# mpc001/auto_avsr

Measured on AMD Instinct MI355X. Metric: video-frames/sec/node (25fps 88x88, max-frames=1600), E2E training step (fwd+bwd+clip+AdamW), higher is better.
Workload: dtype f16 activations x f16x2 weights (atrunk3, atrunk4, decoder, encoder, trunk3, trunk4) + split-bf16 (everything else) forward / bf16 backward

## Files before the change

### auto_avsr_amd/csrc/gemm_core.h

```cpp
#pragma once
#include <algorithm>
#include "prims.h"

namespace avsr_gemm_impl {

struct Params {
    const void* A;
    const void* B;
    const void* B2;
    int lda, ldb;
    int M, N, K;
    int k_chunk;
    const float* bias;
    int act;
    const void* gate;
    int gate_dtype, ldg;
    float gate_scale;
    float drop_p;
    uint64_t seed;
    float alpha;
    const float* alpha_dev;
    const uint64_t* seed_dev;
    const float* resid;
    int ldr;
    void* C;
    void* C2;
    int ldc2;
    int c_dtype, ldc;
    int accumulate;
    int nsplit, batch_h, nbatch;
    long sAb, sAh, sBb, sBh, sCb, sCh;
    int a_skew, skew_off, skew_lim;
    int resid_dtype;
    int cH, cW, cC;
    int cOH, cOW;
    int cKH, cKW, cS, cPH, cPW;
    int cT, cKT, cPT;
    float* colsum;
    float* colstat;
    int colstat_rows;
    float* colsum_a;
    int cN, xcd_order, ncls;
    int k_rot;
    int cls_tile0[5], cls_py[4], cls_px[4], cls_y0[4], cls_x0[4], cls_h[4], cls_w[4], cls_nkh[4], cls_nkw[4];
};

template <class T> struct Raw8;
template <> struct Raw8<bf16_t> {
    bf16x8 v;
    AVSR_DEV void zero() { v = bf16x8{0, 0, 0, 0, 0, 0, 0, 0}; }
    AVSR_DEV void load(const bf16_t* p) { v = *reinterpret_cast<const bf16x8*>(p); }
    AVSR_DEV void set(int e, const bf16_t* p) { v[e] = (short)*p; }
    AVSR_DEV float get(int e) const { return bf2f((bf16_t)v[e]); }
};
template <> struct Raw8<float> {
    f32x4 a, b;
    AVSR_DEV void zero() { a = f32x4{0, 0, 0, 0}; b = a; }
    AVSR_DEV void load(const float* p) {
        a = *reinterpret_cast<const f32x4*>(p);
        b = *reinterpret_cast<const f32x4*>(p + 4);
    }
    AVSR_DEV void set(int e, const float* p) {
        if (e < 4) a[e] = *p; else b[e - 4] = *p;
    }
    AVSR_DEV float get(int e) const { return e < 4 ? a[e] : b[e - 4]; }
};
// ... 556 lines not shown
```

### auto_avsr_amd/csrc/gemm_fast.hip

```cpp
#include "gemm_fast_kernel.h"
#include "gemm_pair.h"
#include "avsr_hip.h"

namespace {

using avsr_gemm_impl::Params;

#define g_tune avsr_tune_knobs

using avsr_fast::FastKernel;

template <int BM, int BN, int STAGES, int CV, int WGM, int WGN, int ABL, int KS, int F16 = 0, int WP = 1>
__global__ __launch_bounds__(64 * WGM * WGN * KS) void gemm_fast_kernel(Params p) {
    AVSR_DYN_SMEM(smem);
    FastKernel<BM, BN, STAGES, CV, WGM, WGN, ABL, KS, F16, WP>::run(p, smem);
}

template <int BM, int BN, int STAGES, int CV = 0, int WGM = 2, int WGN = 2, int ABL = 0, int KS = 1, int F16 = 0, int WP = 1>
void launch_fast(Params& p, int split_k, hipStream_t stream) {
    using K = FastKernel<BM, BN, STAGES, CV, WGM, WGN, ABL, KS, F16, WP>;
    p.k_rot = CV == 0 ? g_tune[7] : 0;
    p.xcd_order = g_tune[1] == 0 ? (CV == 0 && BM == 64 && BN == 64) : (g_tune[1] == 1);
    int gy;
    if (CV == 0) {
        int kc = (p.K + split_k - 1) / split_k;
        kc = ((kc + 63) / 64) * 64;
        split_k = (p.K + kc - 1) / kc;
        p.k_chunk = kc;
        gy = (p.M + BM - 1) / BM;
    } else {
        split_k = 1;
        int t0 = 0;
        for (int c = 0; c < p.ncls; c++) {
            p.cls_tile0[c] = t0;
            t0 += (int)(((long)p.cN * p.cls_h[c] * p.cls_w[c] + BM - 1) / BM);
        }
        p.cls_tile0[p.ncls] = t0;
        gy = t0;
    }
    dim3 grid((p.N + BN - 1) / BN, gy, split_k), block(K::NTHR);
    AVSR_LAUNCH((gemm_fast_kernel<BM, BN, STAGES, CV, WGM, WGN, ABL, KS, F16, WP>), grid, block, K::LDS_BYTES, stream, p);
}

template <int CV>
bool launch_tile(int tile, Params& p, int split_k, hipStream_t stream) {
    switch (tile) {
        case 1: if (CV == 0) { launch_fast<64, 64, 3, 0>(p, split_k, stream); return true; } return false;
        case 2: launch_fast<128, 64, 3, CV>(p, split_k, stream); return true;
        case 3:
            if (CV == 1 && g_tune[2] == 1) launch_fast<128, 128, 3, 1, 2, 2, 1>(p, split_k, stream);
            else if (CV == 1 && g_tune[2] == 2) launch_fast<128, 128, 3, 1, 2, 2, 2>(p, split_k, stream);
// ... 20 lines not shown

template <int CV>
bool launch_tile_h16(int tile, Params& p, int split_k, hipStream_t stream) {
    switch (tile) {
        case 1: if (CV == 0) { launch_fast<64, 64, 3, 0, 2, 2, 0, 1, 1>(p, split_k, stream); return true; } return false;
        case 4: launch_fast<128, 128, 2, CV, 2, 2, 0, 1, 1>(p, split_k, stream); return true;
        case 7: launch_fast<128, 64, 2, CV, 2, 2, 0, 1, 1>(p, split_k, stream); return true;
        default: return false;
    }
}

template <int CV>
bool launch_tile_h16x2(int tile, Params& p, int split_k, hipStream_t stream) {
    switch (tile) {
        case 1: if (CV == 0) { launch_fast<64, 64, 3, 0, 2, 2, 0, 1, 1, 2>(p, split_k, stream); return true; } return false;
        case 21: if (CV == 0) { launch_fast<64, 64, 2, 0, 2, 2, 0, 1, 1, 2>(p, split_k, stream); return true; } return false;
        case 4: launch_fast<128, 128, 2, CV, 2, 2, 0, 1, 1, 2>(p, split_k, stream); return true;
        case 7: launch_fast<128, 64, 2, CV, 2, 2, 0, 1, 1, 2>(p, split_k, stream); return true;
        case 2: launch_fast<128, 64, 3, CV, 2, 2, 0, 1, 1, 2>(p, split_k, stream); return true;
        case 5: launch_fast<256, 128, 2, CV, 4, 2, 0, 1, 1, 2>(p, split_k, stream); return true;
        case 8: launch_fast<256, 64, 2, CV, 4, 2, 0, 1, 1, 2>(p, split_k, stream); return true;
        case 22: launch_fast<128, 128, 2, CV, 2, 4, 0, 1, 1, 2>(p, split_k, stream); return true;
        case 23: launch_fast<256, 64, 3, CV, 4, 2, 0, 1, 1, 2>(p, split_k, stream); return true;
        case 31: if (CV == 0) { launch_fast<64, 64, 3, 0, 2, 2, 1, 1, 1, 2>(p, split_k, stream); return true; } return false;
        case 32: if (CV == 0) { launch_fast<64, 64, 3, 0, 2, 2, 2, 1, 1, 2>(p, split_k, stream); return true; } return false;
        case 33: if (CV == 0) { launch_fast<128, 64, 2, 0, 2, 2, 1, 1, 1, 2>(p, split_k, stream); return true; } return false;
        case 34: if (CV == 0) { launch_fast<128, 64, 2, 0, 2, 2, 2, 1, 1, 2>(p, split_k, stream); return true; } return false;
        case 35: if (CV == 0) { launch_fast<256, 128, 2, 0, 4, 2, 1, 1, 1, 2>(p, split_k, stream); return true; } return false;
        case 36: if (CV == 0) { launch_fast<256, 128, 2, 0, 4, 2, 2, 1, 1, 2>(p, split_k, stream); return true; } return false;
        default: return false;
    }
}

}

int avsr_conv_patch_supported(int N, int H, int W, int Cg, int Cout_eff, int KH, int KW, int stride, int pad_h, int pad_w);
int avsr_conv_patch_launch(int mode, const void* src, const void* w, const void* w_lo, int ldw, const void* resid, void* out, void* out2,
                           const void* zero_page, int N, int H, int W, int Cg, int Cout_eff, hipStream_t stream);
int avsr_conv3x3_c64_supported(int H, int W);
int avsr_conv3x3_c64_launch(int flip, const void* src, const void* wq, const void* resid, void* out, const void* zero_page, int N,
                            int H, int W, hipStream_t stream);

static int gemm16_nt_impl(int f16, const void* A, int lda, const void* B, const void* B_lo, int ldb, int M, int N, int K, const float* bias,
                          int act, const void* gate, int gate_dtype, int ldg, float gate_scale, float drop_p,
                          uint64_t seed, const uint64_t* seed_dev, float alpha, const float* alpha_dev,
                          const void* resid, int resid_dtype, int ldr, void* C, int c_dtype, int ldc, int accumulate,
                          int split_k, int tile, float* colsum, void* c2, int ldc2, hipStream_t stream) {
    AVSR_REQUIRE(!(colsum && accumulate), "gemm_bf16_nt: colsum needs a non-accumulating output");
    AVSR_REQUIRE(!(accumulate && (act != 0 || gate != nullptr || drop_p > 0.f || resid != nullptr || c2 != nullptr)),
                 f16 ? "gemm_h16_nt: accumulate takes bias and alpha only (no act, gate, dropout, resid or twin)"
                     : "gemm_bf16_nt: accumulate takes bias and alpha only (no act, gate, dropout, resid or twin)");
    AVSR_REQUIRE(K > 0 && K % 64 == 0, "gemm_bf16_nt: K must be a positive multiple of 64");
    AVSR_REQUIRE(lda % 8 == 0 && ldb % 8 == 0, "gemm_bf16_nt: lda/ldb must be multiples of 8 elements");
    AVSR_REQUIRE(((uintptr_t)A % 16) == 0 && ((uintptr_t)B % 16) == 0, "gemm_bf16_nt: operands must be 16-byte aligned");
    AVSR_REQUIRE(!(accumulate && c_dtype != 0), "gemm_bf16_nt: accumulate needs an f32 output");
    AVSR_REQUIRE(!(split_k > 1 && !accumulate), "gemm_bf16_nt: split-K needs accumulate=1");
    if (M <= 0 || N <= 0) return 0;
    Params p{};
    p.A = A; p.B = B; p.B2 = B_lo; p.lda = lda; p.ldb = ldb;
    p.M = M; p.N = N; p.K = K;
    p.bias = bias; p.act = act;
    p.gate = gate; p.gate_dtype = gate_dtype; p.ldg = ldg; p.gate_scale = gate_scale;
    p.drop_p = drop_p; p.seed = seed; p.seed_dev = seed_dev;
    p.alpha = alpha; p.alpha_dev = alpha_dev;
    p.resid = reinterpret_cast<const float*>(resid); p.resid_dtype = resid_dtype; p.ldr = ldr;
    p.C = C; p.c_dtype = c_dtype; p.ldc = ldc; p.accumulate = accumulate;
    p.colsum = colsum;
    AVSR_REQUIRE(c2 == nullptr || (!accumulate && c_dtype != 1), "gemm_*_nt: the bf16 twin needs a non-accumulating f32 / f16 output");
    p.C2 = c2; p.ldc2 = ldc2;
    p.nsplit = 1; p.batch_h = 1; p.nbatch = 1;
    if (split_k < 1) split_k = 1;
    float* colsum_det = nullptr;
    if (avsr_det()) {
        split_k = 1;
        if (colsum) {
            AVSR_REQUIRE(ldc == N, "gemm_*_nt (deterministic mode): colsum needs a dense output");
            colsum_det = colsum;
            p.colsum = nullptr;
        }
    }
    const bool auto_tile = tile == 0;
    if (tile == 0) {
        const long t128 = (long)((M + 127) / 128) * ((N + 127) / 128);
        const long t12864 = (long)((M + 127) / 128) * ((N + 63) / 64);
        tile = t128 >= 1024 ? 4 : (t12864 >= 400 ? 7 : (g_tune[14] > 0 && (long)((M + 63) / 64) * ((N + 63) / 64) > 256 ? g_tune[14] : 1));
    }
    if (f16 && B_lo) {
        AVSR_REQUIRE(((uintptr_t)B_lo % 16) == 0, "gemm_h16_nt: the lo plane must be 16-byte aligned");
        if (auto_tile) {
            const long t12864 = (long)((M + 127) / 128) * ((N + 63) / 64);
            const long t256 = (long)((M + 255) / 256) * ((N + 127) / 128);
            tile = g_tune[17] > 0 ? g_tune[17] : (t256 >= 160 && g_tune[17] == 0 ? 5 : (t12864 >= 256 ? 7 : (K >= 2048 && t12864 >= 128 ? 2 : 1)));
        }
        AVSR_REQUIRE(launch_tile_h16x2<0>(tile, p, split_k, stream), "gemm_h16_nt: unknown tile code (two weight planes)");
        if (colsum_det) avsr_colsum_det(C, c_dtype, ldc, M, N, colsum_det, stream);
        AVSR_CHECK_LAUNCH("gemm_h16_nt");
        return 0;
    }
    if (f16) {
        if (tile != 1 && tile != 4 && tile != 7) tile = 1;
        AVSR_REQUIRE(launch_tile_h16<0>(tile, p, split_k, stream), "gemm_h16_nt: unknown tile code");
        if (colsum_det) avsr_colsum_det(C, c_dtype, ldc, M, N, colsum_det, stream);
        AVSR_CHECK_LAUNCH("gemm_h16_nt");
        return 0;
    }
    if (!avsr_det() && avsr_pair::stash_nt(p, tile, split_k, stream)) return 0;
    AVSR_REQUIRE(launch_tile<0>(tile, p, split_k, stream), "gemm_bf16_nt: unknown tile code");
    if (colsum_det) avsr_colsum_det(C, c_dtype, ldc, M, N, colsum_det, stream);
    AVSR_CHECK_LAUNCH("gemm_bf16_nt");
    return 0;
}

extern "C" int avsr_gemm_bf16_nt(const void* A, int lda, const void* B, int ldb, int M, int N, int K, const float* bias,
                                 int act, const void* gate, int gate_dtype, int ldg, float gate_scale, float drop_p,
                                 uint64_t seed, const uint64_t* seed_dev, float alpha, const float* alpha_dev,
                                 const void* resid, int resid_dtype, int ldr, void* C, int c_dtype, int ldc, int accumulate,
                                 int split_k, int tile, float* colsum, hipStream_t stream) {
    return gemm16_nt_impl(0, A, lda, B, nullptr, ldb, M, N, K, bias, act, gate, gate_dtype, ldg, gate_scale, drop_p, seed, seed_dev, alpha,
                          alpha_dev, resid, resid_dtype, ldr, C, c_dtype, ldc, accumulate, split_k, tile, colsum, nullptr, 0, stream);
}

extern "C" int avsr_gemm_h16_nt(const void* A, int lda, const void* B, const void* B_lo, int ldb, int M, int N, int K, const float* bias,
                                int act, float drop_p, uint64_t seed, const uint64_t* seed_dev, float alpha, const void* resid,
// ... 303 lines not shown
```

### auto_avsr_amd/csrc/gemm_fast_kernel.h

```cpp
#pragma once
#include <type_traits>
#include "gemm_core.h"

namespace avsr_fast {

using avsr_gemm_impl::Params;

template <int BM, int BN, int STAGES, int CV = 0, int WGM = 2, int WGN = 2, int ABL = 0, int KS = 1, int F16 = 0, int WP = 1>
struct FastKernel {
    static_assert(WP == 1 || (WP == 2 && F16 == 1 && KS == 1), "two weight planes: f16 operands only");
    static constexpr int BK = 64, NQ = WGM * WGN, NW = NQ * KS, NTHR = 64 * NW;
    static constexpr int KPG = (BK / 16) / KS;
    static_assert(KS == 1 || KS == 2 || KS == 4, "k-split of the 64-wide tile");
    static constexpr int WM = BM / WGM, WN = BN / WGN, TM = WM / 32, TN = WN / 32;
    static constexpr int A_BYTES = BM * 128, B_BYTES = BN * 128, STAGE_BYTES = A_BYTES + WP * B_BYTES;
    static constexpr int A_LOADS = BM / (8 * NW), B_LOADS = BN / (8 * NW);
    static constexpr int LPT = A_LOADS + WP * B_LOADS;
    static constexpr size_t RING_BYTES = (size_t)STAGES * STAGE_BYTES, EPI_BYTES = (size_t)BM * (BN + 4) * 4;
    static constexpr size_t MAP_OFF = RING_BYTES > EPI_BYTES ? RING_BYTES : EPI_BYTES;
    static constexpr size_t LDS_BYTES = MAP_OFF + (CV == 2 ? BM * 4 : 0);
    static_assert(A_LOADS >= 1 && B_LOADS >= 1 && BM % (8 * NW) == 0 && BN % (8 * NW) == 0, "tile / wave-count mismatch");
    static_assert(WM % 32 == 0 && WN % 32 == 0, "wave tile must be a multiple of 32x32");

    struct Rows {
// ... 204 lines not shown
            for (int ks = 0; ks < KPG; ks++) {
#pragma unroll
                for (int i = 0; i < TM; i++)
#pragma unroll
                    for (int j = 0; j < TN; j++) {
                        acc[i][j] = mfma32x<F16>(fa[ks & 1][i], fb[ks & 1][j], acc[i][j]);
                        if (WP == 2) acc_lo[i][j] = mfma32x<F16>(fa[ks & 1][i], fl[ks & 1][j], acc_lo[i][j]);
                    }
                if (ks + 2 < KPG) load_frags(ks & 1, ks0 + ks + 2);
                sched_fence();
            }
        };
        int t = 0;
        for (; t + STAGES - 1 < nt; t++) step(t, std::true_type{});
        for (; t < nt; t++) step(t, std::false_type{});
        if (WP == 2) {
#pragma unroll
            for (int i = 0; i < TM; i++)
#pragma unroll
                for (int j = 0; j < TN; j++)
#pragma unroll
                    for (int r = 0; r < 16; r++) acc[i][j][r] += acc_lo[i][j][r] * (1.0f / AVSR_H16_LO_SCALE);
        }
        if (CV != 0) {
            Params q = p;
            q.gate = nullptr;
            avsr_gemm_impl::epilogue_lds<BM, BN, TM, TN, NTHR, KS>(acc, q, m0, n0, wm * WM, wn * WN, zs, 0, smem, rowmap, kg);
        } else {
            avsr_gemm_impl::epilogue_lds<BM, BN, TM, TN, NTHR, KS>(acc, p, m0, n0, wm * WM, wn * WN, zs, 0, smem, nullptr, kg);
        }
    }
};

}
```

### auto_avsr_amd/csrc/gemm_pair.hip

```cpp
#include "gemm_fast_kernel.h"
#include "gemm_tn_kernel.h"
#include "gemm_pair.h"
#include "avsr_hip.h"

namespace {

using avsr_gemm_impl::Params;
using avsr_fast::FastKernel;
using Tn = avsr_tn::TnKernel<3, 0>;
using Tn4 = avsr_tn::TnKernel<3, 0, 1, 1, 4>;
using Tn128 = avsr_tn::TnKernel<2, 0, 2, 2>;

struct PairState {
    bool active = false, have_nt = false, have_tn = false;
    Params nt, tn;
    int nt_tile = 0;
    int gxa = 0, gya = 0;
    int gxb = 0, gyb = 0, gzb = 0;
    int tn_big = 0;
    hipStream_t stream = nullptr;
};
thread_local PairState g_pair;

template <class KA, class KB>
__global__ __launch_bounds__(256) void gemm_pair_kernel(Params pa, Params pb, int na, int gxa, int gya, int gxb, int gyb) {
    AVSR_DYN_SMEM(smem);
    int b = blockIdx.x;
    if (b < na) {
        const int by = b / gxa;
        KA::run_at(pa, smem, b - by * gxa, by, 0, gxa, gya, 1);
    } else {
        b -= na;
        const int r = b / gxb;
        KB::run_at(pb, smem, b - r * gxb, r % gyb, r / gyb);
    }
}

template <class KA, class KB>
void launch_pair(const PairState& s) {
    const int na = s.have_nt ? s.gxa * s.gya : 0;
    const int nb = s.have_tn ? s.gxb * s.gyb * s.gzb : 0;
    const size_t lds = KA::LDS_BYTES > KB::LDS_BYTES ? KA::LDS_BYTES : KB::LDS_BYTES;
    AVSR_LAUNCH((gemm_pair_kernel<KA, KB>), dim3(na + nb), dim3(256), lds, s.stream, s.nt, s.tn, na, s.gxa > 0 ? s.gxa : 1,
                s.gya > 0 ? s.gya : 1, s.gxb > 0 ? s.gxb : 1, s.gyb > 0 ? s.gyb : 1);
}

}

namespace avsr_pair {

bool stash_nt(const Params& p, int tile, int split_k, hipStream_t stream) {
    PairState& s = g_pair;
    if (!s.active || s.have_nt || split_k > 1 || p.accumulate || (tile != 1 && tile != 7)) return false;
    if (s.have_tn && s.stream != stream) return false;
    s.nt = p;
    s.nt.xcd_order = (tile == 1 && avsr_tune_knobs[1] != 2) ? 1 : 0;
    s.nt.k_chunk = ((p.K + 63) / 64) * 64;
    s.nt_tile = tile;
    const int BM = tile == 1 ? 64 : 128;
    s.gxa = (p.N + 63) / 64;
    s.gya = (p.M + BM - 1) / BM;
    s.stream = stream;
    s.have_nt = true;
    return true;
}

bool stash_tn(const Params& p, int split_k, hipStream_t stream) {
    PairState& s = g_pair;
    if (!s.active || s.have_tn) return false;
    if (s.have_nt && s.stream != stream) return false;
    if (split_k < 1) split_k = 1;
    int kc = (p.K + split_k - 1) / split_k;
    kc = ((kc + 63) / 64) * 64;
    split_k = (p.K + kc - 1) / kc;
    s.tn = p;
    s.tn_big = avsr_tune_knobs[19] == 2 && p.M >= 128 && p.N >= 128;
    if (s.tn_big) {
        split_k = 1;
        kc = ((p.K + 63) / 64) * 64;
    }
// ... 36 lines not shown
```

### auto_avsr_amd/csrc/loss.hip

```cpp
#include "prims.h"
#include "avsr_hip.h"
#include "ctc_common.h"

namespace {

AVSR_DEV float log_add(float a, float b) {
    const float m = fmaxf(a, b);
    if (m <= LOG_ZERO) return LOG_ZERO;
    return m + logf(avsr_exp(a - m) + avsr_exp(b - m));
}
AVSR_DEV float log_add3(float a, float b, float c) {
    const float m = fmaxf(a, fmaxf(b, c));
    if (m <= LOG_ZERO) return LOG_ZERO;
    const float sum = avsr_exp(a - m) + avsr_exp(b - m) + avsr_exp(c - m);
#ifdef AVSR_EMU
    return m + logf(sum);
#else
    return m + __logf(sum);
#endif
}

template <class T>
__global__ __launch_bounds__(256) void row_lse_kernel(const T* __restrict__ x, long ld, float* __restrict__ lse,
                                                      long rows, int V) {
// ... 305 lines not shown

__global__ __launch_bounds__(256) void embed_fwd_kernel(const int64_t* __restrict__ ids, const float* __restrict__ table,
                                                        const float* __restrict__ pe, float* __restrict__ out, long rows,
                                                        int L, int D, float scale, float p, uint64_t seed0,
                                                        const uint64_t* seed_dev) {
    const uint64_t seed = seed0 + (seed_dev ? *seed_dev : 0ull);
    const float inv_keep = p > 0.f ? 1.f / (1.f - p) : 1.f;
    const int dv = D >> 3;
    for (long i = (long)blockIdx.x * 256 + threadIdx.x; i < rows * dv; i += (long)gridDim.x * 256) {
        const long r = i / dv;
        const int c = (int)(i % dv) * 8;
        float e[8], q[8], o[8];
        load8(table + ids[r] * D + c, e);
        load8(pe + (r % L) * D + c, q);
#pragma unroll
        for (int k = 0; k < 8; k++)
            o[k] = (e[k] * scale + q[k]) * dropout_scale(seed, (uint64_t)(r * D + c + k), p, inv_keep);
        store8(out + r * D + c, o);
    }
}
__global__ __launch_bounds__(256) void embed_bwd_kernel(const int64_t* __restrict__ ids, const float* __restrict__ dout,
                                                        float* __restrict__ dtable, long rows, int D, float scale,
                                                        float p, uint64_t seed0, const uint64_t* seed_dev) {
    const uint64_t seed = seed0 + (seed_dev ? *seed_dev : 0ull);
    const float inv_keep = p > 0.f ? 1.f / (1.f - p) : 1.f;
    for (long i = (long)blockIdx.x * 256 + threadIdx.x; i < rows * D; i += (long)gridDim.x * 256) {
        const long r = i / D;
        const int c = (int)(i % D);
        const int64_t id = ids[r];
        bool first = true;
        for (long q = 0; q < r; q++)
            if (ids[q] == id) {
                first = false;
                break;
            }
        if (!first) continue;
        float g = 0.f;
        for (long q = r; q < rows; q++)
            if (ids[q] == id) g += dout[q * D + c] * scale * dropout_scale(seed, (uint64_t)(q * D + c), p, inv_keep);
        dtable[id * D + c] += g;
    }
}

}

extern "C" int avsr_row_lse(const void* x, int dtype, int64_t ld, float* lse, int64_t rows, int V, hipStream_t stream) {
    AVSR_REQUIRE(ld % 8 == 0, "row_lse: ld must be a multiple of 8");
    if (rows <= 0) return 0;
    dim3 grid((unsigned)((rows + 3) / 4)), block(256);
    if (dtype == 0) AVSR_LAUNCH((row_lse_kernel<float>), grid, block, 0, stream, (const float*)x, (long)ld, lse, (long)rows, V);
    else AVSR_LAUNCH((row_lse_kernel<bf16_t>), grid, block, 0, stream, (const bf16_t*)x, (long)ld, lse, (long)rows, V);
    AVSR_CHECK_LAUNCH("row_lse");
    return 0;
}

extern "C" int64_t avsr_ctc_workspace_bytes(int B, int T, int Lmax) {
    const int64_t Smax = 2 * (int64_t)Lmax + 1;
    return ((int64_t)B * T * (1 + 3 * Smax)) * 4 + ((int64_t)B * Smax + B) * 4 + 64;
}

extern "C" int avsr_ctc_loss(const void* logits, int dtype, int64_t ld, const int64_t* labels, int Lmax, int ignore_id,
                             const int64_t* in_lens, float* nll, void* grad, int64_t ldg, void* workspace, int B, int T,
                             int V, hipStream_t stream) {
// ... 62 lines not shown
                                    int64_t* ys_in, int64_t* ys_out, uint8_t* mask, int64_t* n_tokens, hipStream_t stream) {
    AVSR_REQUIRE(L >= 1 && L <= 4096, "prepare_targets: label width out of range");
    if (B <= 0) return 0;
    const size_t lds = (size_t)2 * L * sizeof(int64_t) + ((L + 1 + 7) / 8) * 8;
    AVSR_LAUNCH(prepare_targets_kernel, dim3(B), dim3(256), lds, stream, ys_pad, B, L, sos, eos, ignore_id, ys_in, ys_out, mask, n_tokens);
    AVSR_CHECK_LAUNCH("prepare_targets");
    return 0;
}

extern "C" int avsr_embed_fwd(const int64_t* ids, const float* table, const float* pe, float* out, int64_t rows, int L,
                              int D, float scale, float drop_p, uint64_t seed, const uint64_t* seed_dev, hipStream_t stream) {
    AVSR_REQUIRE(D % 8 == 0, "embed: D must be a multiple of 8");
    if (rows <= 0) return 0;
    long nb = (rows * (D >> 3) + 255) / 256;
    AVSR_LAUNCH(embed_fwd_kernel, dim3((unsigned)(nb > 4096 ? 4096 : nb)), dim3(256), 0, stream, ids, table, pe, out, (long)rows, L, D, scale,
                drop_p, seed, seed_dev);
    AVSR_CHECK_LAUNCH("embed_fwd");
    return 0;
}

extern "C" int avsr_embed_bwd(const int64_t* ids, const float* dout, float* dtable, int64_t rows, int D, float scale,
                              float drop_p, uint64_t seed, const uint64_t* seed_dev, hipStream_t stream) {
    if (rows <= 0) return 0;
    long nb = (rows * D + 255) / 256;
    AVSR_LAUNCH(embed_bwd_kernel, dim3((unsigned)(nb > 4096 ? 4096 : nb)), dim3(256), 0, stream, ids, dout, dtable, (long)rows, D, scale, drop_p,
                seed, seed_dev);
    AVSR_CHECK_LAUNCH("embed_bwd");
    return 0;
}

extern "C" int avsr_log_softmax(const float* x, int64_t ld, float* lse_ws, float* out, int64_t rows, int V,
                                hipStream_t stream) {
    if (rows <= 0) return 0;
    int rc = avsr_row_lse(x, 0, ld, lse_ws, rows, V, stream);
    if (rc) return rc;
    AVSR_LAUNCH(sub_row_scalar_kernel, dim3((unsigned)rows), dim3(256), 0, stream, x, (long)ld, lse_ws, out, (long)rows, V);
    AVSR_CHECK_LAUNCH("log_softmax");
    return 0;
}
```

### auto_avsr_amd/csrc/prims.h

```cpp
#pragma once

extern "C" void avsr_note_launch(int err);
extern "C" int avsr_take_launch_error(void);
#ifdef AVSR_EMU
#include "hip_emu.h"
#define AVSR_LAUNCH(kern, grid, block, smem, stream, ...) \
    emu::launch((grid), (block), (smem), [=]() { kern(__VA_ARGS__); })
#define AVSR_DYN_SMEM(name) char* name = emu::dyn_smem()
#else
#include <hip/hip_runtime.h>
#define AVSR_LAUNCH(kern, grid, block, smem, stream, ...)                          \
    do {                                                                           \
        (void)hipGetLastError();                                                   \
        hipLaunchKernelGGL(kern, (grid), (block), (smem), (stream), __VA_ARGS__);  \
        avsr_note_launch((int)hipGetLastError());                                  \
    } while (0)
#define AVSR_DYN_SMEM(name) extern __shared__ __attribute__((aligned(16))) char name[]
#endif

#include <stdint.h>

#define AVSR_DEV __device__ __forceinline__
#define AVSR_WAVE 64

// ... 110 lines not shown
    __builtin_amdgcn_s_barrier();
#endif
}
AVSR_DEV int wave_id() {
#ifdef AVSR_EMU
    return (int)(threadIdx.x >> 6);
#else
    return __builtin_amdgcn_readfirstlane((int)(threadIdx.x >> 6));
#endif
}
AVSR_DEV void sched_fence() {
#ifndef AVSR_EMU
    __builtin_amdgcn_sched_barrier(0);
#endif
}
template <class T> AVSR_DEV void reg_opaque(T& v) {
#ifndef AVSR_EMU
    asm volatile("" : "+v"(v));
#endif
}
template <int N> AVSR_DEV void wait_vmcnt() {
#ifndef AVSR_EMU
    asm volatile("s_waitcnt vmcnt(%0)" ::"n"(N) : "memory");
#endif
}

AVSR_DEV bf16x4 lds_tr16(const bf16_t* p) {
#ifdef AVSR_EMU
    bf16x4 mine = *reinterpret_cast<const bf16x4*>(p);
    size_t stride;
    const unsigned char* all = emu::wave_gather(&mine, sizeof(mine), &stride);
    const int l = emu::lane_id(), i = l & 15, g = l >> 4;
    bf16x4 out;
    for (int j = 0; j < 4; j++) {
        bf16x4 src;
        memcpy(&src, all + (size_t)(16 * g + 4 * j + (i >> 2)) * stride, sizeof(src));
        out[j] = src[i & 3];
    }
    return out;
#else
    return __builtin_amdgcn_ds_read_tr16_b64_v4i16((__attribute__((address_space(3))) bf16x4*)p);
#endif
}

AVSR_DEV bf16x4 lds_tr16_async(const bf16_t* p) {
#ifdef AVSR_EMU
// ... 299 lines not shown
```

### auto_avsr_amd/ops.py

```python
import contextlib
import math
import os

import torch

from . import _lib

F32, BF16, F16 = 0, 1, 2
_DT = {torch.float32: F32, torch.bfloat16: BF16, torch.float16: F16}
NT, NN, TN = 0, 1, 2


def dt(t, split8_ok=False):
    if isinstance(t, Split8):
        if not split8_ok:
            raise TypeError("a split8-layout activation reached an entry point that cannot read it")
        return 3
    return _DT[t.dtype]


def _ptr(t):
    return None if t is None else t.data_ptr()


# ... 50 lines not shown

def _nb(*ts):
    return float(sum(t.numel() * t.element_size() for t in ts if t is not None))


SPLIT_FAST = os.environ.get("AVSR_SPLIT_FAST", "1") != "0"
PAIR_GEMMS = os.environ.get("AVSR_PAIR_GEMMS", "1") != "0"


@contextlib.contextmanager
def paired():
    global _pair_cur, _in_pair
    if not PAIR_GEMMS or PROFILE is not None or RECORD is not None:
        _in_pair += 1
        try:
            yield
        finally:
            _in_pair -= 1
        return
    L = _lib.lib()
    if PAIR_RECORD is not None:
        _pair_cur = []
    L.call("avsr_gemm_pair_begin")
    try:
        yield
    finally:
        L.call("avsr_gemm_pair_end")
        if PAIR_RECORD is not None and _pair_cur is not None:
            PAIR_RECORD.append(_pair_cur)
        _pair_cur = None


TWIN = None


def _twin(y):
    return TWIN(y) if (TWIN is not None and y.dtype in (torch.float32, torch.float16)) else None


def layernorm_fwd(x, gamma, beta, out_dtype, eps=1e-12, twin=False):
    rows, cols = x.numel() // x.shape[-1], x.shape[-1]
    y = torch.empty(x.shape, dtype=out_dtype, device=x.device)
    mean = torch.empty(rows, dtype=torch.float32, device=x.device)
    rstd = torch.empty(rows, dtype=torch.float32, device=x.device)
    y2 = _twin(y) if twin else None
    if out_dtype == torch.float16:
        call("avsr_layernorm_fwd_h16", _ptr(x), _ptr(gamma), _ptr(beta), _ptr(y), _ptr(y2), _ptr(mean), _ptr(rstd), rows, cols, eps,
             _stream(x), nbytes=_nb(x, y, y2))
        return y, mean, rstd
    if y2 is not None:
        call("avsr_layernorm_fwd2", _ptr(x), _ptr(gamma), _ptr(beta), _ptr(y), _ptr(y2), _ptr(mean), _ptr(rstd), rows, cols, eps,
             _stream(x), nbytes=_nb(x, y, y2))
        return y, mean, rstd
# ... 758 lines not shown


def maxpool2d_bwd(idx, dy, N, H, W, C, K, S, P):
    dx = torch.empty(N, H, W, C, dtype=dy.dtype, device=dy.device)
    call("avsr_maxpool2d_bwd", _ptr(idx), _ptr(dy), _ptr(dx), dt(dy), N, H, W, C, K, S, P, _stream(dy), nbytes=_nb(idx, dy, dx))
    return dx


def avgpool_fwd(x, groups, win, C):
    y = torch.empty(groups, C, dtype=torch.float32, device=x.device)
    call("avsr_avgpool_fwd", _ptr(x), dt(x), _ptr(y), groups, win, C, _stream(x))
    return y


def avgpool_bwd(dy, out_dtype, groups, win, C):
    dx = torch.empty(groups * win, C, dtype=out_dtype, device=dy.device)
    call("avsr_avgpool_bwd", _ptr(dy), _ptr(dx), dt(dx), groups, win, C, _stream(dy))
    return dx


def gemm_bf16_nt(A, lda, B, ldb, M, N, K, C, ldc, *, bias=None, act=0, gate=None, ldg=0, gate_scale=1.0, drop_p=0.0,
                 seed=0, seed_dev=None, alpha=1.0, alpha_dev=None, resid=None, ldr=0, accumulate=False, split_k=1,
                 tile=0, colsum=None):
    call("avsr_gemm_bf16_nt", _ptr(A), lda, _ptr(B), ldb, M, N, K, _ptr(bias), act, _ptr(gate),
         dt(gate) if gate is not None else 0, ldg, gate_scale, drop_p, seed, _ptr(seed_dev), alpha, _ptr(alpha_dev),
         _ptr(resid), dt(resid) if resid is not None else 0, ldr, _ptr(C), dt(C), ldc, int(accumulate), split_k, tile,
         _ptr(colsum), _stream(A), flops=2.0 * M * N * K,
         nbytes=2.0 * (M * K + N * K) + float(M * N * C.element_size()) + (float(M * N * resid.element_size()) if resid is not None else 0.0)
         + (2.0 * M * N if gate is not None else 0.0))
    return C


def gemm_f32s_nt(A, lda, B, ldb, M, N, K, C, ldc, *, bias=None, act=0, gate=None, ldg=0, gate_scale=1.0, drop_p=0.0,
                 seed=0, seed_dev=None, alpha=1.0, alpha_dev=None, resid=None, ldr=0, accumulate=False, split_k=1,
                 tile=0, colsum=None, twin=False):
    c2 = _twin(C) if (twin and not accumulate and C.dtype == torch.float32 and C.dim() == 2 and C.stride(0) == ldc and C.is_contiguous()) else None
    call("avsr_gemm_f32s_nt", _ptr(A), lda, _ptr(B), ldb, M, N, K, _ptr(bias), act, _ptr(gate),
         dt(gate) if gate is not None else 0, ldg, gate_scale, drop_p, seed, _ptr(seed_dev), alpha, _ptr(alpha_dev),
         _ptr(resid), dt(resid) if resid is not None else 0, ldr, _ptr(C), dt(C), ldc, int(accumulate), split_k, tile,
         _ptr(colsum), int(isinstance(B, Split8)), _ptr(c2), ldc, _stream(A), flops=2.0 * M * N * K,
         nbytes=4.0 * (M * K + N * K) + float(M * N * C.element_size()) + (float(M * N * resid.element_size()) if resid is not None else 0.0))
    return C


def gemm_h16_nt(A, lda, B, ldb, M, N, K, C, ldc, *, bias=None, act=0, drop_p=0.0, seed=0, seed_dev=None, alpha=1.0,
                resid=None, ldr=0, tile=0, twin=False, B_lo=None):
    assert A.dtype == torch.float16 and B.dtype == torch.float16 and (B_lo is None or B_lo.dtype == torch.float16)
    c2 = _twin(C) if (twin and C.dtype in (torch.float16, torch.float32) and C.dim() == 2 and C.stride(0) == ldc and C.is_contiguous()) else None
    call("avsr_gemm_h16_nt", _ptr(A), lda, _ptr(B), _ptr(B_lo), ldb, M, N, K, _ptr(bias), act, drop_p, seed, _ptr(seed_dev), alpha,
         _ptr(resid), dt(resid) if resid is not None else 0, ldr, _ptr(C), dt(C), ldc, tile, _ptr(c2), ldc, _stream(A),
         flops=2.0 * M * N * K,
         nbytes=2.0 * (M * K + (2 if B_lo is not None else 1) * N * K) + float(M * N * C.element_size())
         + (float(M * N * resid.element_size()) if resid is not None else 0.0) + (2.0 * M * N if c2 is not None else 0.0))
    return C


def transpose_cast(src, R, Ccols, ld_src=None, pad_to=64):
    ldd = (R + pad_to - 1) // pad_to * pad_to
    dst = torch.empty(Ccols, ldd, dtype=torch.bfloat16, device=src.device)
    call("avsr_transpose_cast", _ptr(src), dt(src), ld_src or Ccols, _ptr(dst), ldd, R, Ccols, _stream(src))
    return dst


def cast_transpose_colsum(src, R, Ccols, *, ld_src=None, want_dst=False, want_T=True, colsum=None, alpha=1.0,
                          alpha_dev=None, drop_p=0.0, seed=0, seed_dev=None):
    dst = torch.empty(R, Ccols, dtype=torch.bfloat16, device=src.device) if want_dst else None
    ldd = (R + 63) // 64 * 64
    dstT = torch.empty(Ccols, ldd, dtype=torch.bfloat16, device=src.device) if want_T else None
    call("avsr_cast_transpose_colsum", _ptr(src), dt(src), ld_src or Ccols, _ptr(dst), _ptr(dstT), ldd, _ptr(colsum), R,
         Ccols, alpha, _ptr(alpha_dev), drop_p, seed, _ptr(seed_dev), _stream(src))
    return dst, dstT
# ... 62 lines not shown
```

### include/avsr_hip.h

```cpp
#ifndef AVSR_HIP_H
#define AVSR_HIP_H
#include <stdint.h>

#if defined(__HIP__) || defined(AVSR_EMU)
typedef hipStream_t avsr_stream_t;
#else
typedef void* avsr_stream_t;
#endif

#ifdef __cplusplus
extern "C" {
#endif

int avsr_abi_version(void);
int avsr_is_emulator(void);
const char* avsr_last_error(void);

int avsr_layernorm_fwd(const float* x, const float* gamma, const float* beta, void* y, int y_dtype,
                       float* mean, float* rstd, int rows, int cols, float eps,
                       avsr_stream_t stream);
int avsr_layernorm_fwd2(const float* x, const float* gamma, const float* beta, float* y, void* y2, float* mean, float* rstd,
                        int rows, int cols, float eps, avsr_stream_t stream);
int avsr_layernorm_bwd(const void* dy, int dy_dtype, const float* x, const float* gamma,
                       const float* mean, const float* rstd, const float* dres, float* dx,
// ... 227 lines not shown
                        avsr_stream_t stream);

int avsr_cast_transpose_colsum(const void* src, int src_dtype, int64_t ld_src, void* dst, void* dstT, int64_t ld_dstT,
                               float* colsum, int R, int C, float alpha, const float* alpha_dev, float drop_p,
                               uint64_t seed, const uint64_t* seed_dev, avsr_stream_t stream);

int avsr_multi_cast_transpose(const void* table, int n, int total_blocks, avsr_stream_t stream);

int64_t avsr_stem357_workspace_bytes(void);
int avsr_stem357_fwd(const float* x, const float* w, void* y, void* workspace, int B, int T, int H, int W,
                     avsr_stream_t stream);
int avsr_stem357_wgrad(const void* dy, const float* x, float* dw, void* workspace, int B, int T, int H, int W,
                       avsr_stream_t stream);
int avsr_stem357_fwd_f32s(const float* x, const float* w, float* y, void* y2 , void* workspace,
                          int B, int T, int H, int W, avsr_stream_t stream);
int64_t avsr_stem357_stat_rows(int B, int T, int H);
int avsr_stem357_fwd_f32s_stats(const float* x, const float* w, float* y, void* y2, void* workspace, int B, int T, int H, int W,
                                float* stats_part, int stats_rows, avsr_stream_t stream);

int avsr_gemm_bf16_tn(const void* A, int lda, const void* B, int ldb, int M, int N, int K, float* C, int ldc,
                      int accumulate, int split_k, const void* zero_page, float* colsum_a, avsr_stream_t stream);
int avsr_gemm_pair_begin(void);
int avsr_gemm_pair_end(void);
int avsr_conv2d_wgrad_bf16(const void* dy, const void* x, float* dwp, const void* zero_page, int N, int H, int W,
                           int Cin, int Cout, int KH, int KW, int stride, int pad_h, int pad_w,
                           avsr_stream_t stream);
int64_t avsr_conv3x3_wgrad_workspace_bytes(int N, int H, int W, int Cin, int Cout, int stride);
int avsr_conv3x3_wgrad_bf16(const void* dy, const void* x, float* dwp, const void* zero_page, void* workspace,
                            int64_t workspace_bytes, int N, int H, int W, int Cin, int Cout, int stride,
                            int torch_layout ,
                            avsr_stream_t stream);
int avsr_ctc_prefix_score(const float* logp, int T, int V, int ldv, const float* r_prev, const int64_t* last,
                          const int64_t* cand, int NH, int S, int out_len, int blank, float* r_new, float* psi,
                          float* psi_eos, avsr_stream_t stream);
int avsr_ctc_prefix_score_batch(int U, const float* const* logp, const int32_t* T, const int32_t* ldv, int V, const float* r_prev,
                                const int64_t* last, const int64_t* cand, const int32_t* row_off, const int32_t* n_rows,
                                const int64_t* frame_off, int pitch, int S, int out_len, int blank, float* r_new, float* psi,
                                float* psi_eos, avsr_stream_t stream);

int64_t avsr_beam_create(const int32_t* cfg, const float* fcfg, const void* const* w, int n_w);
int avsr_beam_destroy(int64_t handle);
int avsr_beam_attach_lm(int64_t handle, const int32_t* cfg, const float* fcfg, const void* const* w, int n_w);
#define AVSR_BIAS_MAX_NODES (1 << 24)
#define AVSR_BIAS_MAX_EDGES (1 << 24)
int avsr_bias_score(const int32_t* first, const int32_t* tok, const int32_t* child, const int32_t* unc, int n_nodes, int n_edges,
                    const int32_t* node, const int64_t* cand, int n, int S, int eos, float* gain, int32_t* next, avsr_stream_t stream);
// ... 80 lines not shown
```

Before: 70330.

## Add in-kernel split-K with ticket reduction and parallelize embedding backward

Adds an automatic split-K path for small-tile-count, long-K GEMMs. Each K-slice writes fp32 partials to a workspace slab, and the last block to arrive (found through an atomic ticket counter) sums the slices and runs the epilogue. This is meant to fill more CUs on GEMMs whose output grid is small. The pair-kernel launcher is extended to handle split-K slices, and new 4- and 6-stage 64x64 tile variants are added. Separately, the embedding backward is rewritten to use one block per row, with a parallel duplicate check and prefix-scan compaction, replacing a quadratic serial scan per element. Costs include the extra slab traffic, a counter-clear launch, and a per-call Python workspace allocation.

Measured after the change: 70730 (median of 6 runs). No clear change (+0.6%).

```diff
diff --git a/auto_avsr_amd/csrc/gemm_core.h b/auto_avsr_amd/csrc/gemm_core.h
--- a/auto_avsr_amd/csrc/gemm_core.h
+++ b/auto_avsr_amd/csrc/gemm_core.h
@@ -42,6 +42,9 @@
     float* colsum_a;
     int cN, xcd_order, ncls;
     int k_rot;
+    float* sk_slab;
+    int* sk_cnt;
+    int sk_n;
     int cls_tile0[5], cls_py[4], cls_px[4], cls_y0[4], cls_x0[4], cls_h[4], cls_w[4], cls_nkh[4], cls_nkw[4];
 };
 
diff --git a/auto_avsr_amd/csrc/gemm_fast.hip b/auto_avsr_amd/csrc/gemm_fast.hip
--- a/auto_avsr_amd/csrc/gemm_fast.hip
+++ b/auto_avsr_amd/csrc/gemm_fast.hip
@@ -27,6 +27,7 @@
         kc = ((kc + 63) / 64) * 64;
         split_k = (p.K + kc - 1) / kc;
         p.k_chunk = kc;
+        p.sk_n = p.sk_slab ? split_k : 1;
         gy = (p.M + BM - 1) / BM;
     } else {
         split_k = 1;
@@ -93,6 +94,8 @@
         case 8: launch_fast<256, 64, 2, CV, 4, 2, 0, 1, 1, 2>(p, split_k, stream); return true;
         case 22: launch_fast<128, 128, 2, CV, 2, 4, 0, 1, 1, 2>(p, split_k, stream); return true;
         case 23: launch_fast<256, 64, 3, CV, 4, 2, 0, 1, 1, 2>(p, split_k, stream); return true;
+        case 24: if (CV == 0) { launch_fast<64, 64, 4, 0, 2, 2, 0, 1, 1, 2>(p, split_k, stream); return true; } return false;
+        case 25: if (CV == 0) { launch_fast<64, 64, 6, 0, 2, 2, 0, 1, 1, 2>(p, split_k, stream); return true; } return false;
         case 31: if (CV == 0) { launch_fast<64, 64, 3, 0, 2, 2, 1, 1, 1, 2>(p, split_k, stream); return true; } return false;
         case 32: if (CV == 0) { launch_fast<64, 64, 3, 0, 2, 2, 2, 1, 1, 2>(p, split_k, stream); return true; } return false;
         case 33: if (CV == 0) { launch_fast<128, 64, 2, 0, 2, 2, 1, 1, 1, 2>(p, split_k, stream); return true; } return false;
@@ -112,11 +115,104 @@
 int avsr_conv3x3_c64_launch(int flip, const void* src, const void* wq, const void* resid, void* out, const void* zero_page, int N,
                             int H, int W, hipStream_t stream);
 
+namespace {
+
+int resolve_tile(int family, int tile, int M, int N, int K) {
+    const bool auto_tile = tile == 0;
+    if (tile == 0) {
+        const long t128 = (long)((M + 127) / 128) * ((N + 127) / 128);
+        const long t12864 = (long)((M + 127) / 128) * ((N + 63) / 64);
+        tile = t128 >= 1024 ? 4 : (t12864 >= 400 ? 7 : (g_tune[14] > 0 && (long)((M + 63) / 64) * ((N + 63) / 64) > 256 ? g_tune[14] : 1));
+    }
+    if (family == 2) {
+        if (auto_tile) {
+            const long t12864 = (long)((M + 127) / 128) * ((N + 63) / 64);
+            const long t256 = (long)((M + 255) / 256) * ((N + 127) / 128);
+            tile = g_tune[17] > 0 ? g_tune[17] : (t256 >= 160 && g_tune[17] == 0 ? 5 : (t12864 >= 256 ? 7 : (K >= 2048 && t12864 >= 128 ? 2 : 1)));
+        }
+    } else if (family == 1) {
+        if (tile != 1 && tile != 4 && tile != 7) tile = 1;
+    }
+    return tile;
+}
+
+bool tile_shape(int tile, int& bm, int& bn) {
+    switch (tile) {
+        case 1: case 9: case 10: case 14: case 15: case 21: case 24: case 25: case 31: case 32: bm = 64; bn = 64; return true;
+        case 2: case 7: case 11: case 12: case 33: case 34: bm = 128; bn = 64; return true;
+        case 3: case 4: case 13: case 22: bm = 128; bn = 128; return true;
+        case 5: case 6: case 35: case 36: bm = 256; bn = 128; return true;
+        case 8: case 23: bm = 256; bn = 64; return true;
+        default: return false;
+    }
+}
+
+int splitk_slices(int tile, int M, int N, int K, long* tiles_out) {
+    int bm, bn;
+    if (tiles_out) *tiles_out = 0;
+    if (!tile_shape(tile, bm, bn) || M <= 0 || N <= 0 || K < 64) return 1;
+    const long tiles = (long)((M + bm - 1) / bm) * ((N + bn - 1) / bn);
+    if (tiles_out) *tiles_out = tiles;
+    const int knob = g_tune[29], kt = K / 64;
+    if (knob == 1 || avsr_det()) return 1;
+    int s;
+    if (knob >= 2) s = knob;
+    else {
+        if (tiles > 96 || kt < 32) return 1;
+        s = std::min(kt / 16, 3);
+    }
+    s = std::max(1, std::min(s, kt));
+    const int per = (kt + s - 1) / s;
+    return (kt + per - 1) / per;
+}
+
+__global__ __launch_bounds__(256) void splitk_clear_kernel(int* __restrict__ cnt, int n) {
+    const int i = blockIdx.x * 256 + threadIdx.x;
+    if (i < n) cnt[i] = 0;
+}
+
+struct SplitkArm {
+    void* slabs = nullptr;
+    int64_t slab_bytes = 0;
+    void* counters = nullptr;
+    int64_t n_counters = 0;
+    int clear = 1;
+};
+thread_local SplitkArm g_sk_arm;
+
+}
+
+extern "C" int64_t avsr_gemm_splitk_workspace_bytes(int family, int M, int N, int K, int tile) {
+    if (K <= 0 || K % 64 != 0) return 0;
+    const int t = resolve_tile(family, tile, M, N, K);
+    long tiles = 0;
+    const int s = splitk_slices(t, M, N, K, &tiles);
+    int bm = 0, bn = 0;
+    if (s <= 1 || !tile_shape(t, bm, bn)) return 0;
+    return (int64_t)tiles * s * bm * bn * 4;
+}
+extern "C" int64_t avsr_gemm_splitk_counters(int family, int M, int N, int K, int tile) {
+    if (K <= 0 || K % 64 != 0) return 0;
+    long tiles = 0;
+    const int s = splitk_slices(resolve_tile(family, tile, M, N, K), M, N, K, &tiles);
+    return s > 1 ? tiles : 0;
+}
+extern "C" int avsr_gemm_splitk_arm(void* slabs, int64_t slab_bytes, void* counters, int64_t n_counters, int clear) {
+    AVSR_REQUIRE(slabs != nullptr && counters != nullptr && ((uintptr_t)slabs % 16) == 0 && ((uintptr_t)counters % 4) == 0,
+                 "gemm_splitk_arm: slabs (16-byte aligned) and counters required");
+    g_sk_arm.slabs = slabs; g_sk_arm.slab_bytes = slab_bytes;
+    g_sk_arm.counters = counters; g_sk_arm.n_counters = n_counters;
+    g_sk_arm.clear = clear;
+    return 0;
+}
+
 static int gemm16_nt_impl(int f16, const void* A, int lda, const void* B, const void* B_lo, int ldb, int M, int N, int K, const float* bias,
                           int act, const void* gate, int gate_dtype, int ldg, float gate_scale, float drop_p,
                           uint64_t seed, const uint64_t* seed_dev, float alpha, const float* alpha_dev,
                           const void* resid, int resid_dtype, int ldr, void* C, int c_dtype, int ldc, int accumulate,
                           int split_k, int tile, float* colsum, void* c2, int ldc2, hipStream_t stream) {
+    const SplitkArm arm = g_sk_arm;
+    g_sk_arm = SplitkArm{};
     AVSR_REQUIRE(!(colsum && accumulate), "gemm_bf16_nt: colsum needs a non-accumulating output");
     AVSR_REQUIRE(!(accumulate && (act != 0 || gate != nullptr || drop_p > 0.f || resid != nullptr || c2 != nullptr)),
                  f16 ? "gemm_h16_nt: accumulate takes bias and alpha only (no act, gate, dropout, resid or twin)"
@@ -150,26 +246,30 @@
             p.colsum = nullptr;
         }
     }
-    const bool auto_tile = tile == 0;
-    if (tile == 0) {
-        const long t128 = (long)((M + 127) / 128) * ((N + 127) / 128);
-        const long t12864 = (long)((M + 127) / 128) * ((N + 63) / 64);
-        tile = t128 >= 1024 ? 4 : (t12864 >= 400 ? 7 : (g_tune[14] > 0 && (long)((M + 63) / 64) * ((N + 63) / 64) > 256 ? g_tune[14] : 1));
-    }
-    if (f16 && B_lo) {
+    const int family = f16 ? (B_lo ? 2 : 1) : 0;
+    tile = resolve_tile(family, tile, M, N, K);
+    if (arm.slabs && !accumulate && split_k == 1) {
+        long tiles = 0;
+        const int s = splitk_slices(tile, M, N, K, &tiles);
+        int bm = 0, bn = 0;
+        if (s > 1 && tile_shape(tile, bm, bn)) {
+            AVSR_REQUIRE(arm.slab_bytes >= (int64_t)tiles * s * bm * bn * 4 && arm.n_counters >= tiles,
+                         "gemm_*_nt: the armed split-K workspace is smaller than avsr_gemm_splitk_workspace_bytes / _counters");
+            p.sk_slab = reinterpret_cast<float*>(arm.slabs);
+            p.sk_cnt = reinterpret_cast<int*>(arm.counters);
+            split_k = s;
+            if (arm.clear)
+                AVSR_LAUNCH(splitk_clear_kernel, dim3((unsigned)((tiles + 255) / 256)), dim3(256), 0, stream, p.sk_cnt, (int)tiles);
+        }
+    }
+    if (family == 2) {
         AVSR_REQUIRE(((uintptr_t)B_lo % 16) == 0, "gemm_h16_nt: the lo plane must be 16-byte aligned");
-        if (auto_tile) {
-            const long t12864 = (long)((M + 127) / 128) * ((N + 63) / 64);
-            const long t256 = (long)((M + 255) / 256) * ((N + 127) / 128);
-            tile = g_tune[17] > 0 ? g_tune[17] : (t256 >= 160 && g_tune[17] == 0 ? 5 : (t12864 >= 256 ? 7 : (K >= 2048 && t12864 >= 128 ? 2 : 1)));
-        }
         AVSR_REQUIRE(launch_tile_h16x2<0>(tile, p, split_k, stream), "gemm_h16_nt: unknown tile code (two weight planes)");
         if (colsum_det) avsr_colsum_det(C, c_dtype, ldc, M, N, colsum_det, stream);
         AVSR_CHECK_LAUNCH("gemm_h16_nt");
         return 0;
     }
-    if (f16) {
-        if (tile != 1 && tile != 4 && tile != 7) tile = 1;
+    if (family == 1) {
         AVSR_REQUIRE(launch_tile_h16<0>(tile, p, split_k, stream), "gemm_h16_nt: unknown tile code");
         if (colsum_det) avsr_colsum_det(C, c_dtype, ldc, M, N, colsum_det, stream);
         AVSR_CHECK_LAUNCH("gemm_h16_nt");
diff --git a/auto_avsr_amd/csrc/gemm_fast_kernel.h b/auto_avsr_amd/csrc/gemm_fast_kernel.h
--- a/auto_avsr_amd/csrc/gemm_fast_kernel.h
+++ b/auto_avsr_amd/csrc/gemm_fast_kernel.h
@@ -250,12 +250,59 @@
 #pragma unroll
                     for (int r = 0; r < 16; r++) acc[i][j][r] += acc_lo[i][j][r] * (1.0f / AVSR_H16_LO_SCALE);
         }
+        int zs_epi = zs;
+        if (CV == 0 && KS == 1 && p.sk_n > 1) {
+            constexpr int NV = TM * TN * 4;
+            const int tile = by * gx_ + bx;
+            f32x4* slab = reinterpret_cast<f32x4*>(p.sk_slab) + (size_t)tile * p.sk_n * (NV * NTHR) + threadIdx.x;
+            f32x4* mine = slab + (size_t)zs * (NV * NTHR);
+#pragma unroll
+            for (int i = 0; i < TM; i++)
+#pragma unroll
+                for (int j = 0; j < TN; j++)
+#pragma unroll
+                    for (int q = 0; q < 4; q++)
+                        mine[((i * TN + j) * 4 + q) * NTHR] =
+                            f32x4{acc[i][j][4 * q], acc[i][j][4 * q + 1], acc[i][j][4 * q + 2], acc[i][j][4 * q + 3]};
+            wait_vmcnt<0>();
+            __syncthreads();
+            int* flag = reinterpret_cast<int*>(smem);
+            if (threadIdx.x == 0) {
+                const int ticket = ticket_publish(p.sk_cnt + tile);
+                if (ticket == p.sk_n - 1) ticket_acquire();
+                *flag = ticket;
+            }
+            __syncthreads();
+            if (*flag != p.sk_n - 1) return;
+            f32x16 own[TM][TN];
+#pragma unroll
+            for (int i = 0; i < TM; i++)
+#pragma unroll
+                for (int j = 0; j < TN; j++) own[i][j] = acc[i][j];
+            for (int z = 0; z < p.sk_n; z++) {
+                const f32x4* src = slab + (size_t)z * (NV * NTHR);
+                const bool mine_z = z == zs;
+#pragma unroll
+                for (int i = 0; i < TM; i++)
+#pragma unroll
+                    for (int j = 0; j < TN; j++)
+#pragma unroll
+                        for (int q = 0; q < 4; q++) {
+                            f32x4 v;
+                            if (mine_z) v = f32x4{own[i][j][4 * q], own[i][j][4 * q + 1], own[i][j][4 * q + 2], own[i][j][4 * q + 3]};
+                            else v = src[((i * TN + j) * 4 + q) * NTHR];
+#pragma unroll
+                            for (int e = 0; e < 4; e++) acc[i][j][4 * q + e] = z == 0 ? v[e] : acc[i][j][4 * q + e] + v[e];
+                        }
+            }
+            zs_epi = 0;
+        }
         if (CV != 0) {
             Params q = p;
             q.gate = nullptr;
             avsr_gemm_impl::epilogue_lds<BM, BN, TM, TN, NTHR, KS>(acc, q, m0, n0, wm * WM, wn * WN, zs, 0, smem, rowmap, kg);
         } else {
-            avsr_gemm_impl::epilogue_lds<BM, BN, TM, TN, NTHR, KS>(acc, p, m0, n0, wm * WM, wn * WN, zs, 0, smem, nullptr, kg);
+            avsr_gemm_impl::epilogue_lds<BM, BN, TM, TN, NTHR, KS>(acc, p, m0, n0, wm * WM, wn * WN, zs_epi, 0, smem, nullptr, kg);
         }
     }
 };
diff --git a/auto_avsr_amd/csrc/gemm_pair.hip b/auto_avsr_amd/csrc/gemm_pair.hip
--- a/auto_avsr_amd/csrc/gemm_pair.hip
+++ b/auto_avsr_amd/csrc/gemm_pair.hip
@@ -27,8 +27,9 @@
     AVSR_DYN_SMEM(smem);
     int b = blockIdx.x;
     if (b < na) {
-        const int by = b / gxa;
-        KA::run_at(pa, smem, b - by * gxa, by, 0, gxa, gya, 1);
+        const int per = gxa * gya, bz = b / per, t = b - bz * per;
+        const int by = t / gxa;
+        KA::run_at(pa, smem, t - by * gxa, by, bz, gxa, gya, pa.sk_n);
     } else {
         b -= na;
         const int r = b / gxb;
@@ -38,7 +39,7 @@
 
 template <class KA, class KB>
 void launch_pair(const PairState& s) {
-    const int na = s.have_nt ? s.gxa * s.gya : 0;
+    const int na = s.have_nt ? s.gxa * s.gya * (s.nt.sk_n > 1 ? s.nt.sk_n : 1) : 0;
     const int nb = s.have_tn ? s.gxb * s.gyb * s.gzb : 0;
     const size_t lds = KA::LDS_BYTES > KB::LDS_BYTES ? KA::LDS_BYTES : KB::LDS_BYTES;
     AVSR_LAUNCH((gemm_pair_kernel<KA, KB>), dim3(na + nb), dim3(256), lds, s.stream, s.nt, s.tn, na, s.gxa > 0 ? s.gxa : 1,
@@ -51,11 +52,16 @@
 
 bool stash_nt(const Params& p, int tile, int split_k, hipStream_t stream) {
     PairState& s = g_pair;
-    if (!s.active || s.have_nt || split_k > 1 || p.accumulate || (tile != 1 && tile != 7)) return false;
+    if (!s.active || s.have_nt || (split_k > 1 && !p.sk_slab) || p.accumulate || (tile != 1 && tile != 7)) return false;
     if (s.have_tn && s.stream != stream) return false;
     s.nt = p;
     s.nt.xcd_order = (tile == 1 && avsr_tune_knobs[1] != 2) ? 1 : 0;
-    s.nt.k_chunk = ((p.K + 63) / 64) * 64;
+    {
+        int kc = (p.K + split_k - 1) / split_k;
+        kc = ((kc + 63) / 64) * 64;
+        s.nt.k_chunk = kc;
+        s.nt.sk_n = p.sk_slab ? (p.K + kc - 1) / kc : 1;
+    }
     s.nt_tile = tile;
     const int BM = tile == 1 ? 64 : 128;
     s.gxa = (p.N + 63) / 64;
diff --git a/auto_avsr_amd/csrc/loss.hip b/auto_avsr_amd/csrc/loss.hip
--- a/auto_avsr_amd/csrc/loss.hip
+++ b/auto_avsr_amd/csrc/loss.hip
@@ -351,23 +351,61 @@
 __global__ __launch_bounds__(256) void embed_bwd_kernel(const int64_t* __restrict__ ids, const float* __restrict__ dout,
                                                         float* __restrict__ dtable, long rows, int D, float scale,
                                                         float p, uint64_t seed0, const uint64_t* seed_dev) {
+    __shared__ int s_dup;
+    __shared__ int s_wave[4];
+    __shared__ int s_list[256];
     const uint64_t seed = seed0 + (seed_dev ? *seed_dev : 0ull);
     const float inv_keep = p > 0.f ? 1.f / (1.f - p) : 1.f;
-    for (long i = (long)blockIdx.x * 256 + threadIdx.x; i < rows * D; i += (long)gridDim.x * 256) {
-        const long r = i / D;
-        const int c = (int)(i % D);
-        const int64_t id = ids[r];
-        bool first = true;
-        for (long q = 0; q < r; q++)
-            if (ids[q] == id) {
-                first = false;
-                break;
+    const long r = blockIdx.x;
+    const int tid = threadIdx.x, lane = tid & 63, wave = tid >> 6;
+    const int64_t id = ids[r];
+    if (tid == 0) s_dup = 0;
+    __syncthreads();
+    bool dup = false;
+    for (long q = tid; q < r; q += 256) dup |= ids[q] == id;
+    if (dup) s_dup = 1;
+    __syncthreads();
+    if (s_dup) return;
+    constexpr int CPT = 4;
+    for (int c0 = 0; c0 < D; c0 += 256 * CPT) {
+        float g[CPT];
+#pragma unroll
+        for (int k = 0; k < CPT; k++) g[k] = 0.f;
+        for (long base = r; base < rows; base += 256) {
+            const long q = base + tid;
+            const int hit = (q < rows && ids[q] == id) ? 1 : 0;
+            int incl = hit;
+#pragma unroll
+            for (int d = 1; d < 64; d <<= 1) {
+                const int up = __shfl_up(incl, d);
+                if (lane >= d) incl += up;
             }
-        if (!first) continue;
-        float g = 0.f;
-        for (long q = r; q < rows; q++)
-            if (ids[q] == id) g += dout[q * D + c] * scale * dropout_scale(seed, (uint64_t)(q * D + c), p, inv_keep);
-        dtable[id * D + c] += g;
+            __syncthreads();
+            if (lane == 63) s_wave[wave] = incl;
+            __syncthreads();
+            int off = 0, n = 0;
+#pragma unroll
+            for (int w = 0; w < 4; w++) {
+                if (w < wave) off += s_wave[w];
+                n += s_wave[w];
+            }
+            if (hit) s_list[off + incl - 1] = (int)(q - base);
+            __syncthreads();
+            for (int i = 0; i < n; i++) {
+                const long qq = base + s_list[i];
+#pragma unroll
+                for (int k = 0; k < CPT; k++) {
+                    const int c = c0 + k * 256 + tid;
+                    if (c < D) g[k] += dout[qq * D + c] * scale * dropout_scale(seed, (uint64_t)(qq * D + c), p, inv_keep);
+                }
+            }
+        }
+#pragma unroll
+        for (int k = 0; k < CPT; k++) {
+            const int c = c0 + k * 256 + tid;
+            if (c < D) dtable[id * D + c] += g[k];
+        }
+        __syncthreads();
     }
 }
 
@@ -476,9 +514,8 @@
 extern "C" int avsr_embed_bwd(const int64_t* ids, const float* dout, float* dtable, int64_t rows, int D, float scale,
                               float drop_p, uint64_t seed, const uint64_t* seed_dev, hipStream_t stream) {
     if (rows <= 0) return 0;
-    long nb = (rows * D + 255) / 256;
-    AVSR_LAUNCH(embed_bwd_kernel, dim3((unsigned)(nb > 4096 ? 4096 : nb)), dim3(256), 0, stream, ids, dout, dtable, (long)rows, D, scale, drop_p,
-                seed, seed_dev);
+    AVSR_REQUIRE(rows < (1l << 31), "embed_bwd: row count exceeds the grid");
+    AVSR_LAUNCH(embed_bwd_kernel, dim3((unsigned)rows), dim3(256), 0, stream, ids, dout, dtable, (long)rows, D, scale, drop_p, seed, seed_dev);
     AVSR_CHECK_LAUNCH("embed_bwd");
     return 0;
 }
diff --git a/auto_avsr_amd/csrc/prims.h b/auto_avsr_amd/csrc/prims.h
--- a/auto_avsr_amd/csrc/prims.h
+++ b/auto_avsr_amd/csrc/prims.h
@@ -156,6 +156,25 @@
 template <int N> AVSR_DEV void wait_vmcnt() {
 #ifndef AVSR_EMU
     asm volatile("s_waitcnt vmcnt(%0)" ::"n"(N) : "memory");
+#endif
+}
+
+AVSR_DEV int ticket_publish(int* cnt) {
+#ifdef AVSR_EMU
+    __atomic_thread_fence(__ATOMIC_RELEASE);
+    return atomicAdd(cnt, 1);
+#else
+    __builtin_amdgcn_fence(__ATOMIC_RELEASE, "agent");
+    asm volatile("s_waitcnt vmcnt(0)" ::: "memory");
+    return __hip_atomic_fetch_add(cnt, 1, __ATOMIC_RELAXED, __HIP_MEMORY_SCOPE_AGENT);
+#endif
+}
+AVSR_DEV void ticket_acquire() {
+#ifdef AVSR_EMU
+    __atomic_thread_fence(__ATOMIC_ACQUIRE);
+#else
+    __builtin_amdgcn_fence(__ATOMIC_ACQUIRE, "agent");
+    asm volatile("s_waitcnt vmcnt(0)" ::: "memory");
 #endif
 }
 
diff --git a/auto_avsr_amd/ops.py b/auto_avsr_amd/ops.py
--- a/auto_avsr_amd/ops.py
+++ b/auto_avsr_amd/ops.py
@@ -96,13 +96,37 @@
     if PAIR_RECORD is not None:
         _pair_cur = []
     L.call("avsr_gemm_pair_begin")
+    _sk_keep.append(None)
     try:
         yield
     finally:
         L.call("avsr_gemm_pair_end")
+        del _sk_keep[:]
         if PAIR_RECORD is not None and _pair_cur is not None:
             PAIR_RECORD.append(_pair_cur)
         _pair_cur = None
+
+
+SPLITK_WS = None
+_sk_keep = []
+
+
+def _splitk_arm(family, A, M, N, K, tile):
+    L = _lib.lib()
+    nb = L.call("avsr_gemm_splitk_workspace_bytes", family, M, N, K, tile)
+    if not nb:
+        return None
+    nc = L.call("avsr_gemm_splitk_counters", family, M, N, K, tile)
+    if SPLITK_WS is not None:
+        slabs, cnt = SPLITK_WS(nb, nc, A.device)
+    else:
+        slabs = torch.empty(nb // 4, dtype=torch.float32, device=A.device)
+        cnt = zeros_f32((nc,), A.device)
+    captured = SPLITK_WS is None and A.is_cuda and torch.cuda.is_current_stream_capturing()
+    L.call("avsr_gemm_splitk_arm", _ptr(slabs), nb, _ptr(cnt), nc, 0 if captured else 1)
+    if _sk_keep:
+        _sk_keep.append((slabs, cnt))
+    return slabs, cnt
 
 
 TWIN = None
@@ -907,6 +931,7 @@
 def gemm_bf16_nt(A, lda, B, ldb, M, N, K, C, ldc, *, bias=None, act=0, gate=None, ldg=0, gate_scale=1.0, drop_p=0.0,
                  seed=0, seed_dev=None, alpha=1.0, alpha_dev=None, resid=None, ldr=0, accumulate=False, split_k=1,
                  tile=0, colsum=None):
+    ws = _splitk_arm(0, A, M, N, K, tile) if (not accumulate and split_k == 1) else None
     call("avsr_gemm_bf16_nt", _ptr(A), lda, _ptr(B), ldb, M, N, K, _ptr(bias), act, _ptr(gate),
          dt(gate) if gate is not None else 0, ldg, gate_scale, drop_p, seed, _ptr(seed_dev), alpha, _ptr(alpha_dev),
          _ptr(resid), dt(resid) if resid is not None else 0, ldr, _ptr(C), dt(C), ldc, int(accumulate), split_k, tile,
@@ -932,6 +957,7 @@
                 resid=None, ldr=0, tile=0, twin=False, B_lo=None):
     assert A.dtype == torch.float16 and B.dtype == torch.float16 and (B_lo is None or B_lo.dtype == torch.float16)
     c2 = _twin(C) if (twin and C.dtype in (torch.float16, torch.float32) and C.dim() == 2 and C.stride(0) == ldc and C.is_contiguous()) else None
+    ws = _splitk_arm(2 if B_lo is not None else 1, A, M, N, K, tile)
     call("avsr_gemm_h16_nt", _ptr(A), lda, _ptr(B), _ptr(B_lo), ldb, M, N, K, _ptr(bias), act, drop_p, seed, _ptr(seed_dev), alpha,
          _ptr(resid), dt(resid) if resid is not None else 0, ldr, _ptr(C), dt(C), ldc, tile, _ptr(c2), ldc, _stream(A),
          flops=2.0 * M * N * K,
diff --git a/include/avsr_hip.h b/include/avsr_hip.h
--- a/include/avsr_hip.h
+++ b/include/avsr_hip.h
@@ -273,6 +273,9 @@
                       int accumulate, int split_k, const void* zero_page, float* colsum_a, avsr_stream_t stream);
 int avsr_gemm_pair_begin(void);
 int avsr_gemm_pair_end(void);
+int64_t avsr_gemm_splitk_workspace_bytes(int family, int M, int N, int K, int tile);
+int64_t avsr_gemm_splitk_counters(int family, int M, int N, int K, int tile);
+int avsr_gemm_splitk_arm(void* slabs, int64_t slab_bytes, void* counters, int64_t n_counters, int clear);
 int avsr_conv2d_wgrad_bf16(const void* dy, const void* x, float* dwp, const void* zero_page, int N, int H, int W,
                            int Cin, int Cout, int KH, int KW, int stride, int pad_h, int pad_w,
                            avsr_stream_t stream);
```
